# Kainmueller-Lab/PatchPerPix

Measured on AMD Instinct MI355X. Metric: Mvoxels/sec assembled (vote_instances), higher is better.
Workload: dtype f16 in, f32 accumulate

## Files before the change

### patchperpix_amd/csrc/ppp_consensus_v3.hip

```cpp
#include <algorithm>

#include "ppp_kernels.hpp"

namespace ppp {

typedef float v2f __attribute__((ext_vector_type(2)));
typedef float v4f __attribute__((ext_vector_type(4)));
typedef const volatile __attribute__((address_space(3))) v4f *lds_v4f_cvp;

static constexpr int V3_WAVES = 1;
static constexpr int S1V3_GROUP = 3;
static constexpr bool s1v3_prefetch(int PX) { return PX >= 9; }
static constexpr int s1v3_minwaves(int PX) { return PX <= 7 ? 3 : 2; }

static constexpr bool s1v3_split(int PX) { return PX <= 7; }
static constexpr int S1V3_CGROUP = 3;

template <int PX, bool FLAT>
struct V3 {
    static constexpr int RX = PX / 2;
    static constexpr int NC = 64 + (FLAT ? 2 : 1) * (PX - 1);
    static constexpr int NT = 64 + (FLAT ? 4 : 2) * (PX - 1);
    static constexpr int NACC = 2 * PX - 1;
    static constexpr int NEL = PX * NC;
    static constexpr int NIT = (NEL + 63) / 64;
    static constexpr int NELP = NIT * 64;
    static constexpr int FOLD = 255 / PX;
};

__device__ __forceinline__ v2f pk_mul_clamp(v2f a, v2f b) {
    v2f d;
    asm("v_pk_mul_f32 %0, %1, %2 clamp" : "=v"(d) : "v"(a), "v"(b));
    return d;
}
__device__ __forceinline__ v2f pk_fma_clamp(v2f a, v2f b, v2f c) {
    v2f d;
    asm("v_pk_fma_f32 %0, %1, %2, %3 clamp" : "=v"(d) : "v"(a), "v"(b), "v"(c));
    return d;
}
__device__ __forceinline__ v2f pk_nadd_clamp(v2f a, v2f c) {
    v2f d;
    asm("v_pk_add_f32 %0, %1, %2 neg_lo:[1,0] neg_hi:[1,0] clamp" : "=v"(d) : "v"(a), "v"(c));
    return d;
}
__device__ __forceinline__ v2f pk_fma(v2f a, v2f b, v2f c) { return __builtin_elementwise_fma(a, b, c); }
__device__ __forceinline__ uint32_t pk_mad_u16(uint32_t a, uint32_t b, uint32_t c) {
    uint32_t d;
    asm("v_pk_mad_u16 %0, %1, %2, %3" : "=v"(d) : "v"(a), "v"(b), "v"(c));
    return d;
}
__device__ __forceinline__ v2f splat(float x) { return (v2f){x, x}; }
__device__ __forceinline__ uint32_t pack_codes(v2f pos, v2f neg) {
    const v2f c = pk_fma(neg, splat(256.0f), pos);
    return (uint32_t)c.x | ((uint32_t)c.y << 16);
}

template <int PX, int NC, bool ROW0, bool EXACT>
__device__ __forceinline__ void tile_votes3(const v2f *at, const v2f *cfp, lds_v4f_cvp bt, const v2f *bt2, const uint32_t *ct,
                                            const double th2, const double den,
                                            v2f (&acc)[2 * PX - 1], uint32_t (&tc)[2 * PX - 1]) {
    const v2f kq = splat(-0.25f), c43 = splat(0x1.555556p+0f), c43lo = splat(-0x1.555556p-25f);
    constexpr int GS = S1V3_GROUP;
    constexpr int NJG = (PX + GS - 1) / GS;
    constexpr int NG = PX * NJG;
    v4f bcur[GS], bnxt[GS];
    v2f ta, ta_nxt, fa, fa_nxt, ga, na;
    uint32_t ca = 0u;
    lds_v4f_cvp btg[GS];
#pragma unroll
    for (int g = 0; g < GS; ++g) btg[g] = bt;
    auto used = [](int kx, int j) { return j < PX && !(ROW0 && j <= kx); };
    auto load_group = [&](int n, v4f (&b)[GS], v2f &t, v2f &f) {
        const int kx = PX - 1 - n / NJG, jg = (n % NJG) * GS;
        if (jg == 0) { t = at[kx * NC - kx]; f = cfp[-kx]; }
#pragma unroll
        for (int g = 0; g < GS; ++g)
            if (used(kx, jg + g)) {
                if constexpr (s1v3_split(PX)) {
                    const v2f t2 = bt2[(jg + g) * NC - kx];
                    b[g] = (v4f){t2.x, t2.y, __uint_as_float(ct[(jg + g) * NC - kx]), 0.0f};
                } else {
                    b[g] = btg[g][(jg + g) * NC - kx];
                }
            }
    };
    load_group(0, bcur, ta, fa);
#pragma unroll
    for (int n = 0; n < NG; ++n) {
        const int kx = PX - 1 - n / NJG, jg = (n % NJG) * GS;
        if (n + 1 < NG) load_group(n + 1, bnxt, ta_nxt, fa_nxt);
        if (jg == 0) {
            if constexpr (EXACT) ta = (v2f){fa.x != 0.0f ? ta.x : 0.0f, fa.y != 0.0f ? ta.y : 0.0f};
            else ta = ta * fa;
            if constexpr (!EXACT) {
                ga = pk_mul_clamp(ta, splat(4.0f));
                na = pk_mul_clamp(ta, splat(-4.0f));
            } else {
                ga = (v2f){ta.x > 0.0f ? 1.0f : 0.0f, ta.y > 0.0f ? 1.0f : 0.0f};
                na = (v2f){ta.x < 0.0f ? 1.0f : 0.0f, ta.y < 0.0f ? 1.0f : 0.0f};
            }
            ca = pack_codes(ga, na);
        }
        v2f tb[GS], x[GS], y[GS];
        uint32_t cb[GS];
#pragma unroll
        for (int g = 0; g < GS; ++g) {
            if (!used(kx, jg + g)) continue;
            tb[g] = (v2f){bcur[g].x, bcur[g].y};
            cb[g] = __float_as_uint(bcur[g].z);
            x[g] = ta * tb[g];
        }
        if constexpr (!EXACT) {
            v2f dp[GS], dn[GS], d[GS], q0[GS];
#pragma unroll
            for (int g = 0; g < GS; ++g) if (used(kx, jg + g)) dp[g] = pk_fma_clamp(x[g], ga, kq);
#pragma unroll
            for (int g = 0; g < GS; ++g) if (used(kx, jg + g)) dn[g] = pk_nadd_clamp(x[g], kq);
#pragma unroll
            for (int g = 0; g < GS; ++g) if (used(kx, jg + g)) d[g] = dp[g] - dn[g];
#pragma unroll
            for (int g = 0; g < GS; ++g) if (used(kx, jg + g)) q0[g] = d[g] * c43lo;
#pragma unroll
            for (int g = 0; g < GS; ++g) if (used(kx, jg + g)) y[g] = pk_fma(d[g], c43, q0[g]);
        } else {
#pragma unroll
            for (int g = 0; g < GS; ++g) {
                if (!used(kx, jg + g)) continue;
#pragma unroll
                for (int s = 0; s < 2; ++s) {
                    const float a = s ? ta.y : ta.x, b = s ? tb[g].y : tb[g].x, xs = s ? x[g].y : x[g].x;
                    const bool valid = a != 0.0f && b != 0.0f && !(a < 0.0f && b < 0.0f);
                    const double xd = (double)xs;
                    const float ys = (float)((xd - __builtin_copysign(th2, xd)) / den);
                    if (s) y[g].y = valid ? ys : 0.0f; else y[g].x = valid ? ys : 0.0f;
                }
            }
        }
#pragma unroll
        for (int g = 0; g < GS; ++g) {
            if (!used(kx, jg + g)) continue;
            const int i = jg + g - kx + PX - 1;
            acc[i] = acc[i] + y[g];
            tc[i] = pk_mad_u16(ca, cb[g], tc[i]);
        }
        if (n + 1 < NG) {
#pragma unroll
            for (int g = 0; g < GS; ++g) bcur[g] = bnxt[g];
            if ((n + 1) % NJG == 0) { ta = ta_nxt; fa = fa_nxt; }
        }
        __builtin_amdgcn_sched_barrier(0);
    }
}

typedef __amdgpu_buffer_rsrc_t BufRsrc;
__device__ __forceinline__ BufRsrc buf_rsrc(const void *base) {
    return __builtin_amdgcn_make_buffer_rsrc(const_cast<void *>(base), 0, -1, 0x00020000);
}
template <typename T>
__device__ __forceinline__ unsigned buf_ldraw(BufRsrc r, unsigned voff, unsigned soff);
template <>
__device__ __forceinline__ unsigned buf_ldraw<float>(BufRsrc r, unsigned voff, unsigned soff) {
    return __builtin_amdgcn_raw_buffer_load_b32(r, (int)voff, (int)soff, 0);
}
template <>
__device__ __forceinline__ unsigned buf_ldraw<__half>(BufRsrc r, unsigned voff, unsigned soff) {
    return (unsigned)__builtin_amdgcn_raw_buffer_load_b16(r, (int)voff, (int)soff, 0);
}
template <>
__device__ __forceinline__ unsigned buf_ldraw<bf16_t>(BufRsrc r, unsigned voff, unsigned soff) {
    return (unsigned)__builtin_amdgcn_raw_buffer_load_b16(r, (int)voff, (int)soff, 0);
}
template <typename T>
__device__ __forceinline__ unsigned glb_ldraw(const T *base, unsigned voff, unsigned soff);
template <>
__device__ __forceinline__ unsigned glb_ldraw<float>(const float *base, unsigned voff, unsigned soff) {
    asm volatile("" : "+v"(voff));
    return *reinterpret_cast<const unsigned *>(reinterpret_cast<const char *>(base) + soff + voff);
}
template <>
__device__ __forceinline__ unsigned glb_ldraw<__half>(const __half *base, unsigned voff, unsigned soff) {
    asm volatile("" : "+v"(voff));
    return (unsigned)*reinterpret_cast<const unsigned short *>(reinterpret_cast<const char *>(base) + soff + voff);
}
template <>
__device__ __forceinline__ unsigned glb_ldraw<bf16_t>(const bf16_t *base, unsigned voff, unsigned soff) {
    asm volatile("" : "+v"(voff));
    return (unsigned)*reinterpret_cast<const unsigned short *>(reinterpret_cast<const char *>(base) + soff + voff);
}
template <typename T>
__device__ __forceinline__ float widen(unsigned raw);
template <>
__device__ __forceinline__ float widen<float>(unsigned raw) { return __uint_as_float(raw); }
template <>
__device__ __forceinline__ float widen<__half>(unsigned raw) {
    return (float)__builtin_bit_cast(_Float16, (unsigned short)raw);
}
template <>
__device__ __forceinline__ float widen<bf16_t>(unsigned raw) { return __uint_as_float(raw << 16); }

template <typename T>
__device__ __forceinline__ float ldf_at3(const T *base, unsigned byte_off) {
    asm volatile("" : "+v"(byte_off));
    return ldf(reinterpret_cast<const T *>(reinterpret_cast<const char *>(base) + byte_off), 0);
}

enum { V3_DENSE = 0, V3_LIST = 1, V3_ZERO = 2 };

template <typename T, int PX, bool FLAT, bool CLEAN, int MODE = V3_DENSE>
__global__ void __launch_bounds__(64 * V3_WAVES, s1v3_minwaves(PX))
    consensus_v3_kernel(const T *__restrict__ pred, const uint8_t *__restrict__ ov,
                        float *__restrict__ cons, float *__restrict__ cnt_out, const Geo G,
                        const int n_rows, const int runs_per_line, const int bZ2,
                        const long long n_waves, const uint32_t *__restrict__ items) {
    using K = V3<PX, FLAT>;
    constexpr int NIT = K::NIT;
    constexpr bool SPLIT = s1v3_split(PX);
    constexpr bool VOTES = MODE != V3_ZERO;
    __shared__ v4f lds_bt[V3_WAVES][SPLIT || !VOTES ? 1 : K::NELP];
    __shared__ v2f lds_bt2[V3_WAVES][SPLIT && VOTES ? K::NELP : 1];
    __shared__ uint32_t lds_ct[V3_WAVES][SPLIT && VOTES ? K::NELP : 1];
    __shared__ v2f lds_at[V3_WAVES][VOTES ? K::NELP : 1];
    __shared__ v2f lds_cf[V3_WAVES][VOTES ? K::NC : 1];
    __shared__ uint8_t lds_valid[V3_WAVES][2][2][VOTES ? K::NT + 2 : 1];
    const int wave = __builtin_amdgcn_readfirstlane(threadIdx.x >> 6), lane = threadIdx.x & 63;
    long long bid = blockIdx.x;
    {
        const long long nb = gridDim.x, per = nb / 8, main = per * 8;
        if (bid < main) bid = (bid % 8) * per + bid / 8;
    }
    const long long pos = bid * V3_WAVES + wave;
    if (pos >= n_waves) return;
    long long wid_;
    if constexpr (MODE != V3_DENSE) wid_ = (long long)items[pos]; else wid_ = pos;
    const long long wid = wid_;
    const int row = (int)(wid % n_rows);
    long long run = wid / n_rows;
    int dz, dy;
    if (row < G.py) { dz = 0; dy = row; }
    else { const int t = row - G.py; dz = 1 + t / G.wy; dy = t % G.wy - (G.py - 1); }
    const int xr = (int)(run % runs_per_line);
    run /= runs_per_line;
    int uy, uz, ux0, nA;
    if (FLAT) {
        const int flat0 = xr * 64;
        uy = G.cy0 + flat0 / G.cX;
        uz = G.cz0 + 2 * (int)run;
        ux0 = G.cx0 + flat0 % G.cX;
        nA = min(64, G.cX - flat0 % G.cX);
    } else {
        uy = G.cy0 + (int)(run % G.cY);
        uz = G.cz0 + 2 * (int)(run / G.cY);
        ux0 = G.cx0 + xr * 64;
        nA = 64;
    }
    const bool have_s1 = uz + 1 < G.cz0 + G.cZ;
    const bool in_b = FLAT && lane >= nA;
    const bool have_b = FLAT && nA < 64 && uy + 1 < G.cy0 + G.cY;
    const int ux = in_b ? G.cx0 + (lane - nA) : ux0 + lane;
    const int uy_l = in_b ? uy + 1 : uy;
    const bool lane_ok = in_b ? have_b : ux < G.cx0 + G.cX;
    const int pos_l = lane + (PX - 1) + (in_b ? PX - 1 : 0);
    const int wy = uy + dy;
    const bool wy_ok_a = wy >= 0 && wy < G.Y;
    const bool wy_ok_b = have_b && wy + 1 >= 0 && wy + 1 < G.Y;
    const bool wz_ok0 = uz + dz < G.Z, wz_ok1 = have_s1 && uz + 1 + dz < G.Z;
    const bool w_row_ok = (wy_ok_a || wy_ok_b) && (wz_ok0 || wz_ok1);
    const bool row0 = dz == 0 && dy == 0;

    v2f acc[K::NACC];
    uint32_t tc[K::NACC], cnt[K::NACC];
#pragma unroll
    for (int i = 0; i < K::NACC; ++i) { acc[i] = splat(0.0f); tc[i] = 0u; cnt[i] = 0u; }

    const T *mid = pred + (long long)G.mid * G.V;
    const int ntA = nA + 2 * (PX - 1);
    if constexpr (VOTES) {
#pragma unroll
    for (int s = 0; s < 2; ++s) {
        uint8_t *uval = lds_valid[wave][s][0], *wval = lds_valid[wave][s][1];
        const bool s_ok = s == 0 || have_s1;
        const bool wz_ok = s ? wz_ok1 : wz_ok0;
        for (int i = lane; i < K::NT; i += 64) {
            const bool sb = FLAT && i >= ntA;
            const int x = sb ? G.cx0 - (PX - 1) + (i - ntA) : ux0 - (PX - 1) + i;
            const int yy = sb ? uy + 1 : uy, wyy = sb ? wy + 1 : wy;
            bool vu = false, vw = false;
            if (s_ok && x >= 0 && x < G.X && (!sb || have_b)) {
                const long long lu = vox(G, uz + s, yy, x);
                vu = ldf(mid, lu) > G.th_gt && (!G.use_overlap || ov[lu] == 0);
                if (wz_ok && (sb ? wy_ok_b : wy_ok_a)) {
                    const long long lw = vox(G, uz + s + dz, wyy, x);
                    vw = ldf(mid, lw) > G.th_gt && (!G.use_overlap || ov[lw] == 0);
                }
            }
            uval[i] = vu; wval[i] = vw;
        }
    }
    __builtin_amdgcn_fence(__ATOMIC_ACQ_REL, "wavefront");
    __builtin_amdgcn_wave_barrier();
    }

    unsigned el_off[NIT];
    const int ncA = nA + (PX - 1);
    auto centre_x = [&](int i, bool &sb, bool &ok) -> int {
        sb = FLAT && i >= ncA;
        const int iseg = sb ? i - ncA : i;
        const int cx = (sb ? G.cx0 : ux0) - (PX - 1) + K::RX + iseg;
        ok = cx >= K::RX && cx < G.X - K::RX && (!sb || have_b);
        return min(max(cx, 0), G.X - 1) + (sb ? G.X : 0);
    };
#pragma unroll
    for (int it = 0; it < NIT; ++it) {
        const int e = it * 64 + lane;
        const int i = e % K::NC;
        const int j = min(e / K::NC, PX - 1);
        bool sb, ok;
        const int cxc = centre_x(i, sb, ok);
        el_off[it] = (unsigned)(((long long)j * G.V + cxc) * (long long)sizeof(T));
    }
    unsigned cf_off[2];
    unsigned cf_st = 0, cf_sb = 0;
#pragma unroll
    for (int c = 0; c < 2; ++c) {
        const int i = min(lane + 64 * c, K::NC - 1);
        bool sb, ok;
        const int cxc = centre_x(i, sb, ok);
        cf_off[c] = (unsigned)cxc * (unsigned)sizeof(T);
        cf_st |= ((ok && lane + 64 * c < K::NC) ? 1u : 0u) << c;
        cf_sb |= (sb ? 1u : 0u) << c;
    }

    v2f *at = lds_at[wave], *cf = lds_cf[wave];
    v4f *bt = lds_bt[wave];
    v2f *bt2 = lds_bt2[wave];
    uint32_t *ct = lds_ct[wave];

    if (VOTES && w_row_ok) {
        const int kz_hi = min(G.pz - 1, G.pz - 1 - dz), kz_lo = max(0, -dz);
        const int ky_hi = min(G.py - 1, G.py - 1 - dy), ky_lo = max(0, -dy);
        const long long slice = (long long)G.Y * G.X;
        int kz = kz_hi, ky = ky_hi + 1;
        bool row_a_ok = true, row_b_ok = false;
        bool z_ok0 = true, z_ok1 = false;
        auto next_tile = [&](int &z, int &y) -> bool {
            while (true) {
                if (--y < ky_lo) { y = ky_hi; --z; }
                if (z < kz_lo) return false;
                const int cz = uz - z + G.rz, cy = uy - y + G.ry;
                z_ok0 = cz >= G.rz && cz < G.Z - G.rz;
                z_ok1 = have_s1 && cz + 1 >= G.rz && cz + 1 < G.Z - G.rz;
                if (!(z_ok0 || z_ok1)) continue;
                row_a_ok = cy >= G.ry && cy < G.Y - G.ry;
                row_b_ok = have_b && cy + 1 >= G.ry && cy + 1 < G.Y - G.ry;
                if (row_a_ok || row_b_ok) return true;
            }
        };
        unsigned ra[2][NIT], rb[2][NIT], rc[2][2];
        bool lz0 = true, lz1 = false, la = true, lb = false;
        auto load_tile = [&](int z, int y) {
            lz0 = z_ok0; lz1 = z_ok1; la = row_a_ok; lb = row_b_ok;
            const int cz = uz - z + G.rz;
            const long long crow0 = vox(G, z_ok0 ? cz : cz + 1, uy - y + G.ry, 0);
            const unsigned s1 = __builtin_amdgcn_readfirstlane((z_ok1 && z_ok0) ? (unsigned)(slice * (long long)sizeof(T)) : 0u);
            const long long cha = (long long)((z * G.py + y) * PX) * G.V;
            const long long chb = (long long)(((z + dz) * G.py + (y + dy)) * PX) * G.V;
            const BufRsrc qc = buf_rsrc(mid + crow0);
#pragma unroll
            for (int it = 0; it < NIT; ++it) {
                ra[0][it] = glb_ldraw<T>(pred + cha + crow0, el_off[it], 0u);
                ra[1][it] = glb_ldraw<T>(pred + cha + crow0, el_off[it], s1);
                rb[0][it] = glb_ldraw<T>(pred + chb + crow0, el_off[it], 0u);
                rb[1][it] = glb_ldraw<T>(pred + chb + crow0, el_off[it], s1);
            }
#pragma unroll
            for (int c = 0; c < 2; ++c) {
                rc[0][c] = buf_ldraw<T>(qc, cf_off[c], 0u);
                rc[1][c] = buf_ldraw<T>(qc, cf_off[c], s1);
            }
        };
        constexpr bool PREFETCH = s1v3_prefetch(PX);
        const v2f big26 = splat(0x1p26f), nbig26 = splat(-0x1p26f), hb = splat(0x1p25f),
                  nhb = splat(-0x1p25f);
        int n_fold = 0;
        bool have = next_tile(kz, ky);
        if (PREFETCH && have) load_tile(kz, ky);
        while (have) {
            if (!PREFETCH) load_tile(kz, ky);
#pragma unroll
            for (int c = 0; c < 2; ++c) {
                const bool st = (cf_st >> c) & 1u, sb = (cf_sb >> c) & 1u;
                const bool rok = st && (sb ? lb : la);
                v2f f;
                f.x = (rok && lz0 && widen<T>(rc[0][c]) > G.th_gt) ? 1.0f : 0.0f;
                f.y = (rok && lz1 && widen<T>(rc[1][c]) > G.th_gt) ? 1.0f : 0.0f;
                if (lane + 64 * c < K::NC) cf[lane + 64 * c] = f;
            }
            unsigned bigmax = 0u;
            constexpr int CG = S1V3_CGROUP;
#pragma unroll
            for (int it = 0; it < NIT; ++it)
                asm volatile("" : "+v"(ra[0][it]), "+v"(ra[1][it]), "+v"(rb[0][it]), "+v"(rb[1][it]));
            bool any_big = false;
            if constexpr (CLEAN) {
                const v2f c255 = splat(255.0f), one = splat(1.0f);
#pragma unroll
                for (int i0 = 0; i0 < NIT; i0 += CG) {
                    v2f va[CG], vb[CG], ha[CG], hbb[CG], ta[CG], tb[CG], cc[CG];
#pragma unroll
                    for (int q = 0; q < CG; ++q) if (i0 + q < NIT) {
                        va[q] = (v2f){widen<T>(ra[0][i0 + q]), widen<T>(ra[1][i0 + q])};
                        vb[q] = (v2f){widen<T>(rb[0][i0 + q]), widen<T>(rb[1][i0 + q])};
                    }
#pragma unroll
                    for (int q = 0; q < CG; ++q) if (i0 + q < NIT) ha[q] = pk_fma_clamp(va[q], nbig26, hb);
#pragma unroll
                    for (int q = 0; q < CG; ++q) if (i0 + q < NIT) hbb[q] = pk_fma_clamp(vb[q], nbig26, hb);
#pragma unroll
                    for (int q = 0; q < CG; ++q) if (i0 + q < NIT) ta[q] = va[q] - ha[q];
#pragma unroll
                    for (int q = 0; q < CG; ++q) if (i0 + q < NIT) tb[q] = vb[q] - hbb[q];
#pragma unroll
                    for (int q = 0; q < CG; ++q) if (i0 + q < NIT) cc[q] = pk_fma(hbb[q], c255, one);
#pragma unroll
                    for (int q = 0; q < CG; ++q) if (i0 + q < NIT) {
                        const int e = (i0 + q) * 64 + lane;
                        const uint32_t code = (uint32_t)cc[q].x | ((uint32_t)cc[q].y << 16);
                        at[e] = ta[q];
                        if constexpr (SPLIT) { bt2[e] = tb[q]; ct[e] = code; }
                        else bt[e] = (v4f){tb[q].x, tb[q].y, __uint_as_float(code), 0.0f};
                    }
                }
            } else {
#pragma unroll
            for (int i0 = 0; i0 < NIT; i0 += CG) {
                v2f va[CG], vb[CG], ga[CG], ha[CG], gb[CG], hbb[CG], sa[CG], sbb[CG], ta[CG], tb[CG], cc[CG];
#pragma unroll
                for (int q = 0; q < CG; ++q) if (i0 + q < NIT) {
                    va[q] = (v2f){widen<T>(ra[0][i0 + q]), widen<T>(ra[1][i0 + q])};
                    vb[q] = (v2f){widen<T>(rb[0][i0 + q]), widen<T>(rb[1][i0 + q])};
                }
#pragma unroll
                for (int q = 0; q < CG; ++q) if (i0 + q < NIT) ga[q] = pk_fma_clamp(va[q], big26, nhb);
#pragma unroll
                for (int q = 0; q < CG; ++q) if (i0 + q < NIT) ha[q] = pk_fma_clamp(va[q], nbig26, hb);
#pragma unroll
                for (int q = 0; q < CG; ++q) if (i0 + q < NIT) gb[q] = pk_fma_clamp(vb[q], big26, nhb);
#pragma unroll
                for (int q = 0; q < CG; ++q) if (i0 + q < NIT) hbb[q] = pk_fma_clamp(vb[q], nbig26, hb);
#pragma unroll
                for (int q = 0; q < CG; ++q) if (i0 + q < NIT) sa[q] = ga[q] + ha[q];
#pragma unroll
                for (int q = 0; q < CG; ++q) if (i0 + q < NIT) sbb[q] = gb[q] + hbb[q];
#pragma unroll
                for (int q = 0; q < CG; ++q) if (i0 + q < NIT) cc[q] = pk_fma(hbb[q], splat(256.0f), gb[q]);
#pragma unroll
                for (int q = 0; q < CG; ++q) if (i0 + q < NIT) ta[q] = pk_fma(va[q], sa[q], -ha[q]);
#pragma unroll
                for (int q = 0; q < CG; ++q) if (i0 + q < NIT) tb[q] = pk_fma(vb[q], sbb[q], -hbb[q]);
#pragma unroll
                for (int q = 0; q < CG; ++q) if (i0 + q < NIT) {
                    const int e = (i0 + q) * 64 + lane;
                    bigmax = max(bigmax, max(max(__float_as_uint(va[q].x), __float_as_uint(va[q].y)),
                                             max(__float_as_uint(vb[q].x), __float_as_uint(vb[q].y))));
                    const uint32_t code = (uint32_t)cc[q].x | ((uint32_t)cc[q].y << 16);
                    at[e] = ta[q];
                    if constexpr (SPLIT) { bt2[e] = tb[q]; ct[e] = code; }
                    else bt[e] = (v4f){tb[q].x, tb[q].y, __uint_as_float(code), 0.0f};
                }
            }
            any_big = __ballot(bigmax > 0x3F800000u) != 0ull;
            if (any_big) {
#pragma unroll
                for (int it = 0; it < NIT; ++it) {
                    const int e = it * 64 + lane;
                    v2f ta, tb;
                    unsigned code = 0u;
#pragma unroll
                    for (int s = 0; s < 2; ++s) {
                        const float va = widen<T>(ra[s][it]), vb = widen<T>(rb[s][it]);
                        const float xa = va > G.th_gt ? va : (va < G.bg_lt ? va - 1.0f : 0.0f);
                        const float xb = vb > G.th_gt ? vb : (vb < G.bg_lt ? vb - 1.0f : 0.0f);
                        if (s) { ta.y = xa; tb.y = xb; } else { ta.x = xa; tb.x = xb; }
                        code |= (xb > 0.0f ? 1u : (xb < 0.0f ? 256u : 0u)) << (16 * s);
                    }
                    at[e] = ta;
                    if constexpr (SPLIT) { bt2[e] = tb; ct[e] = code; }
                    else bt[e] = (v4f){tb.x, tb.y, __uint_as_float(code), 0.0f};
                }
            }
            }
            __builtin_amdgcn_fence(__ATOMIC_ACQ_REL, "wavefront");
            __builtin_amdgcn_wave_barrier();
            have = next_tile(kz, ky);
            if (PREFETCH && have) load_tile(kz, ky);
            const v2f *ia = at + pos_l;
            lds_v4f_cvp ib = (lds_v4f_cvp)(bt + (SPLIT ? 0 : pos_l));
            const v2f *ib2 = bt2 + (SPLIT ? pos_l : 0);
            const uint32_t *ic = ct + (SPLIT ? pos_l : 0);
            const v2f *icf = cf + pos_l;
            if (CLEAN || !any_big) {
                if (row0) tile_votes3<PX, K::NC, true, false>(ia, icf, ib, ib2, ic, G.th2, G.den, acc, tc);
                else tile_votes3<PX, K::NC, false, false>(ia, icf, ib, ib2, ic, G.th2, G.den, acc, tc);
            } else if constexpr (!CLEAN) {
                if (row0) tile_votes3<PX, K::NC, true, true>(ia, icf, ib, ib2, ic, G.th2, G.den, acc, tc);
                else tile_votes3<PX, K::NC, false, true>(ia, icf, ib, ib2, ic, G.th2, G.den, acc, tc);
            }
            if (++n_fold == K::FOLD) {
                n_fold = 0;
#pragma unroll
                for (int i = 0; i < K::NACC; ++i) {
                    cnt[i] += (tc[i] & 0x00FF00FFu) + ((tc[i] >> 8) & 0x00FF00FFu);
                    tc[i] = 0u;
                }
            }
            __builtin_amdgcn_fence(__ATOMIC_ACQ_REL, "wavefront");
            __builtin_amdgcn_wave_barrier();
        }
    }
    if (!lane_ok) return;
    __builtin_amdgcn_fence(__ATOMIC_ACQ_REL, "wavefront");
    __builtin_amdgcn_wave_barrier();
    const int ti_u = (in_b ? ntA + (lane - nA) : lane) + PX - 1;
#pragma unroll
    for (int s = 0; s < 2; ++s) {
        if (s == 1 && !have_s1) break;
        const uint8_t *uval = lds_valid[wave][s][0], *wval = lds_valid[wave][s][1];
        const bool u_ok = VOTES && uval[ti_u] != 0;
        float val[K::NACC];
#pragma unroll
        for (int i = 0; i < K::NACC; ++i) {
            const int dx = i - (PX - 1);
            val[i] = 0.0f;
            if (dz == 0 && dy == 0 && dx <= 0) continue;
            const unsigned total = cnt[i] + (tc[i] & 0x00FF00FFu) + ((tc[i] >> 8) & 0x00FF00FFu);
            const bool ok = VOTES && u_ok && wval[ti_u + dx] != 0;
            const unsigned n = ok ? ((s ? total >> 16 : total) & 0xFFFFu) : 0u;
            const float a = ok ? (s ? acc[i].y : acc[i].x) : 0.0f;
            const float c = (float)n;
            val[i] = (G.normalise && n != 0u) ? a / c : a;
            if (G.layout != PPP_CONS_VOXEL_MAJOR) {
                const long long o = cons_at(G, dz, dy, dx, uz + s, uy_l, ux);
                if (cons) cons[o] = val[i];
                if (cnt_out) cnt_out[o] = c;
            }
        }
        if (G.layout == PPP_CONS_VOXEL_MAJOR) {
            const int W = (2 * G.pz - 1) * G.wy * G.wx, Lc = (W - 1) / 2;
            const int L0 = (dz * G.wy + dy) * G.wx;
            const long long vu = ((long long)row_slice(G, uz + s) * G.bY + (uy_l - G.by0)) * G.bX + (ux - G.bx0);
            float *pos = cons + vu * W + Lc + L0 - (PX - 1);
            if (row0) {
                pos[PX - 1] = 0.0f;
#pragma unroll
                for (int i = PX; i < K::NACC; ++i) pos[i] = val[i];
            } else {
                typedef float f4u __attribute__((ext_vector_type(4), aligned(4)));
#pragma unroll
                for (int i = 0; i + 4 <= K::NACC; i += 4)
                    *reinterpret_cast<f4u *>(pos + i) = (f4u){val[i], val[i + 1], val[i + 2], val[i + 3]};
#pragma unroll
                for (int i = K::NACC / 4 * 4; i < K::NACC; ++i) pos[i] = val[i];
            }
            const int wz = uz + s + dz, wy2 = uy_l + dy;
            if (wz < G.bz0 + G.bZ && wy2 >= G.by0 && wy2 < G.by0 + G.bY) {
                const long long vw0 = ((long long)row_slice(G, wz) * G.bY + (wy2 - G.by0)) * G.bX + (ux - G.bx0);
#pragma unroll
                for (int i = 0; i < K::NACC; ++i) {
                    const int dx = i - (PX - 1);
                    if (row0 && dx <= 0) continue;
                    const int wx2 = ux + dx;
                    if (wx2 >= G.bx0 && wx2 < G.bx0 + G.bX) cons[(vw0 + dx) * W + Lc - L0 - dx] = val[i];
                }
            }
        }
    }
}

struct VmFaces { long long start[6]; int lo[5][3], ext[5][3]; };
__global__ void __launch_bounds__(256)
    vm_zero_kernel(float *__restrict__ S, const Geo G, const int n_rows, const VmFaces F) {
    const long long t = (long long)blockIdx.x * blockDim.x + threadIdx.x;
    if (t >= F.start[5] * n_rows) return;
    const int row = (int)(t % n_rows);
    const long long fv = t / n_rows;
    int f = 0;
#pragma unroll
    for (int k = 1; k < 5; ++k) f += fv >= F.start[k] ? 1 : 0;
    const long long r = fv - F.start[f];
    const int ex = F.ext[f][2], ey = F.ext[f][1];
    const int bx = F.lo[f][2] + (int)(r % ex), by = F.lo[f][1] + (int)((r / ex) % ey),
              bz = F.lo[f][0] + (int)(r / ((long long)ex * ey));
    int dz, dy;
    if (row < G.py) { dz = 0; dy = row; }
    else { const int q = row - G.py; dz = 1 + q / G.wy; dy = q % G.wy - (G.py - 1); }
    const int W = (2 * G.pz - 1) * G.wy * G.wx, Lc = (W - 1) / 2;
    float *Sv = S + (((long long)bz * G.bY + by) * G.bX + bx) * W;
    const bool line_out = bz - dz < 0 || by - dy < 0 || by - dy >= G.bY;
    const int L0 = (dz * G.wy + dy) * G.wx;
    for (int dx = -(G.px - 1); dx <= G.px - 1; ++dx) {
        if (row == 0 && dx <= 0) continue;
        const int sx = bx - dx;
        if (line_out || sx < 0 || sx >= G.bX) Sv[Lc - L0 - dx] = 0.0f;
    }
}

static hipError_t launch_vm_zero(float *S, const Geo &G, int n_rows, hipStream_t s) {
    VmFaces F{};
    const int gz = std::min(G.pz - 1, G.bZ), gy = std::min(G.py - 1, G.bY), gx = std::min(G.px - 1, G.bX);
    const int lo[5][3] = {{0, 0, 0}, {0, 0, 0}, {0, G.bY - gy, 0}, {0, 0, 0}, {0, 0, G.bX - gx}};
    const int ext[5][3] = {{gz, G.bY, G.bX}, {G.bZ, gy, G.bX}, {G.bZ, gy, G.bX}, {G.bZ, G.bY, gx}, {G.bZ, G.bY, gx}};
    long long acc = 0;
    for (int f = 0; f < 5; ++f) {
        F.start[f] = acc;
        for (int a = 0; a < 3; ++a) { F.lo[f][a] = lo[f][a]; F.ext[f][a] = std::max(ext[f][a], 1); }
        acc += (long long)ext[f][0] * ext[f][1] * ext[f][2];
    }
    F.start[5] = acc;
    const long long nt = acc * n_rows;
    if (nt == 0) return hipSuccess;
    PPP_GRID_CHECK((nt + 255) / 256, 256);
    vm_zero_kernel<<<dim3((unsigned)((nt + 255) / 256)), dim3(256), 0, s>>>(S, G, n_rows, F);
    return hipGetLastError();
}

template <typename T, int PX, bool FLAT, bool CLEAN>
static hipError_t launch_v3f(const T *pred, const uint8_t *ov, float *cons, float *cnt,
                             const Geo &G, hipStream_t s) {
    const int n_rows = (G.pz - 1) * G.wy + G.py;
    const int runs_per_line = FLAT ? (int)(((long long)G.cX * G.cY + 63) / 64) : (G.cX + 63) / 64;
    const int bZ2 = (G.cZ + 1) / 2;
    const long long n_waves = (long long)runs_per_line * (FLAT ? 1 : G.cY) * bZ2 * n_rows;
    const long long n_blocks = (n_waves + V3_WAVES - 1) / V3_WAVES;
    if (n_blocks >= (1ll << 31)) return hipErrorInvalidValue;
    PPP_GRID_CHECK(n_blocks, 64 * V3_WAVES);
    if (((long long)(PX - 1) * G.V + 2ll * G.X) * (long long)sizeof(T) >= (1ll << 32)) return hipErrorNotSupported;
    if (G.layout == PPP_CONS_VOXEL_MAJOR && !G.vm_open) {
        const hipError_t ez = launch_vm_zero(cons, G, n_rows, s);
        if (ez != hipSuccess) return ez;
    }
    consensus_v3_kernel<T, PX, FLAT, CLEAN><<<dim3((unsigned)n_blocks), dim3(64 * V3_WAVES), 0, s>>>(
        pred, ov, cons, cnt, G, n_rows, runs_per_line, bZ2, n_waves, nullptr);
    return hipGetLastError();
}

template <typename T, int PX, bool FLAT, bool CLEAN>
static hipError_t launch_v3f_lists(const T *pred, const uint8_t *ov, float *cons, float *cnt, const Geo &G,
                                   const uint32_t *active, long long n_active, const uint32_t *inactive,
                                   long long n_inactive, hipStream_t s) {
    const int n_rows = (G.pz - 1) * G.wy + G.py;
    const int runs_per_line = FLAT ? (int)(((long long)G.cX * G.cY + 63) / 64) : (G.cX + 63) / 64;
    const int bZ2 = (G.cZ + 1) / 2;
    const long long n_waves = (long long)runs_per_line * (FLAT ? 1 : G.cY) * bZ2 * n_rows;
    if (n_active + n_inactive != n_waves || n_waves >= (1ll << 32)) return hipErrorInvalidValue;
    if (((long long)(PX - 1) * G.V + 2ll * G.X) * (long long)sizeof(T) >= (1ll << 32)) return hipErrorNotSupported;
    if (G.layout == PPP_CONS_VOXEL_MAJOR && !G.vm_open) {
        const hipError_t ez = launch_vm_zero(cons, G, n_rows, s);
        if (ez != hipSuccess) return ez;
    }
    if (n_active > 0) {
        const long long nb = (n_active + V3_WAVES - 1) / V3_WAVES;
        PPP_GRID_CHECK(nb, 64 * V3_WAVES);
        consensus_v3_kernel<T, PX, FLAT, CLEAN, V3_LIST><<<dim3((unsigned)nb), dim3(64 * V3_WAVES), 0, s>>>(
            pred, ov, cons, cnt, G, n_rows, runs_per_line, bZ2, n_active, active);
        const hipError_t e = hipGetLastError();
        if (e != hipSuccess) return e;
    }
    if (n_inactive > 0) {
        const long long nb = (n_inactive + V3_WAVES - 1) / V3_WAVES;
        PPP_GRID_CHECK(nb, 64 * V3_WAVES);
        consensus_v3_kernel<float, PX, FLAT, true, V3_ZERO><<<dim3((unsigned)nb), dim3(64 * V3_WAVES), 0, s>>>(
            nullptr, nullptr, cons, cnt, G, n_rows, runs_per_line, bZ2, n_inactive, inactive);
    }
    return hipGetLastError();
}

static bool v3_flat(const Geo &G) {
    static EnvSwitch sw("PPP_S1_FLAT");
    const char *e = sw.get();
    bool flat = G.cX >= 64 && G.cX % 64 != 0 && G.py >= 3 && G.cY > 1;
    if (e && e[0] == '0') flat = false;
    if (e && e[0] == '1' && G.cX >= 64 && G.py >= 3) flat = true;
    return flat;
}
static bool v3_clean(const Geo &G) {
    static EnvSwitch swc("PPP_S1_CLEAN");
    const char *ec = swc.get();
    return G.pred_clean == 1 && !(ec && ec[0] == '0');
}

V3Items consensus_v3_items(const Geo &G) {
    V3Items I;
    I.flat = v3_flat(G) ? 1 : 0;
    I.n_rows = (G.pz - 1) * G.wy + G.py;
    I.runs_per_line = I.flat ? (int)(((long long)G.cX * G.cY + 63) / 64) : (G.cX + 63) / 64;
    I.bZ2 = (G.cZ + 1) / 2;
    I.n_runs = (long long)I.runs_per_line * (I.flat ? 1 : G.cY) * I.bZ2;
    I.n_items = I.n_runs * I.n_rows;
    return I;
}

template <typename T, int PX>
static hipError_t launch_v3_lists(const T *pred, const uint8_t *ov, float *cons, float *cnt, const Geo &G,
                                  const uint32_t *act, long long na, const uint32_t *ina, long long ni,
                                  hipStream_t s) {
    const bool flat = v3_flat(G);
    const bool clean = v3_clean(G);
    note_consensus_short_form(clean && na > 0 ? 1 : 0);
    if (clean)
        return flat ? launch_v3f_lists<T, PX, true, true>(pred, ov, cons, cnt, G, act, na, ina, ni, s)
                    : launch_v3f_lists<T, PX, false, true>(pred, ov, cons, cnt, G, act, na, ina, ni, s);
    return flat ? launch_v3f_lists<T, PX, true, false>(pred, ov, cons, cnt, G, act, na, ina, ni, s)
                : launch_v3f_lists<T, PX, false, false>(pred, ov, cons, cnt, G, act, na, ina, ni, s);
}

template <typename T, int PX>
static hipError_t launch_v3(const T *pred, const uint8_t *ov, float *cons, float *cnt,
                            const Geo &G, hipStream_t s) {
    const bool flat = v3_flat(G);
    const bool clean = v3_clean(G);
    note_consensus_short_form(clean ? 1 : 0);
    if (clean)
        return flat ? launch_v3f<T, PX, true, true>(pred, ov, cons, cnt, G, s)
                    : launch_v3f<T, PX, false, true>(pred, ov, cons, cnt, G, s);
    return flat ? launch_v3f<T, PX, true, false>(pred, ov, cons, cnt, G, s)
                : launch_v3f<T, PX, false, false>(pred, ov, cons, cnt, G, s);
}

bool consensus_v3_supported(const Geo &G) {
    static EnvSwitch sw("PPP_S1_V3");
    const char *e = sw.get();
    if (e && e[0] == '0') return false;
    return G.value_rule == PPP_VAL_NORM_PROB_PRODUCT && G.th2 == 0.25 && G.den == 0.75 &&
           G.th_gt == 0.5f && G.bg_lt == 0.5f && (G.px == 3 || G.px == 5 || G.px == 7 || G.px == 9);
}

hipError_t launch_consensus_v3(const void *pred, int dtype, const uint8_t *ov, float *cons,
                               float *cnt, const Geo &G, hipStream_t s) {
    if (!consensus_v3_supported(G)) return hipErrorNotSupported;
    if (G.layout == PPP_CONS_VOXEL_MAJOR && (cnt || !cons)) return hipErrorInvalidValue;
#define PPP_V3_CASE(P)                                                                          \
    case P:                                                                                     \
        return with_pred_type(dtype, [&](auto tag) {                                            \
            using T = PPP_PRED_T(tag);                                                          \
            return launch_v3<T, P>((const T *)pred, ov, cons, cnt, G, s);                       \
        });
    switch (G.px) {
        PPP_V3_CASE(3)
        PPP_V3_CASE(5)
        PPP_V3_CASE(7)
        PPP_V3_CASE(9)
    default:
        return hipErrorNotSupported;
    }
#undef PPP_V3_CASE
}

hipError_t launch_consensus_v3_lists(const void *pred, int dtype, const uint8_t *ov, float *cons, float *cnt,
                                     const Geo &G, const uint32_t *active, long long n_active,
                                     const uint32_t *inactive, long long n_inactive, hipStream_t s) {
    if (!consensus_v3_supported(G)) return hipErrorNotSupported;
    if (G.layout == PPP_CONS_VOXEL_MAJOR && (cnt || !cons)) return hipErrorInvalidValue;
#define PPP_V3_CASE(P)                                                                                       \
    case P:                                                                                                  \
        return with_pred_type(dtype, [&](auto tag) {                                                         \
            using T = PPP_PRED_T(tag);                                                                       \
            return launch_v3_lists<T, P>((const T *)pred, ov, cons, cnt, G, active, n_active, inactive,      \
                                         n_inactive, s);                                                     \
        });
    switch (G.px) {
        PPP_V3_CASE(3)
        PPP_V3_CASE(5)
        PPP_V3_CASE(7)
        PPP_V3_CASE(9)
    default:
        return hipErrorNotSupported;
    }
#undef PPP_V3_CASE
}

}
```

Before: 16.28.

## Stage voxel-major consensus results through LDS for coalesced writes; group dense wave order

For larger patch sizes with voxel-major output, each wave writes its per-lane results into LDS. It then cooperatively stores contiguous vector chunks for both the direct and the mirrored (symmetric) offsets instead of doing per-lane strided stores. It also remaps dense wave indices so that groups of runs sharing a row are scheduled together, which should improve cache locality. The change adds LDS traffic and wave barriers, and the rewritten mirror-write logic carries correctness risk.

```diff
diff --git a/patchperpix_amd/csrc/ppp_consensus_v3.hip b/patchperpix_amd/csrc/ppp_consensus_v3.hip
--- a/patchperpix_amd/csrc/ppp_consensus_v3.hip
+++ b/patchperpix_amd/csrc/ppp_consensus_v3.hip
@@ -14,6 +14,8 @@
 static constexpr int s1v3_minwaves(int PX) { return PX <= 7 ? 3 : 2; }
 
 static constexpr bool s1v3_split(int PX) { return PX <= 7; }
+static constexpr bool s1v3_lds_write(int PX) { return PX >= 7; }
+static constexpr int s1v3_group(int PX) { return PX >= 9 ? 32 : PX >= 7 ? 16 : 0; }
 static constexpr int S1V3_CGROUP = 3;
 
 template <int PX, bool FLAT>
@@ -232,6 +234,13 @@
     if (pos >= n_waves) return;
     long long wid_;
     if constexpr (MODE != V3_DENSE) wid_ = (long long)items[pos]; else wid_ = pos;
+    if constexpr (MODE == V3_DENSE && s1v3_group(PX) > 0) {
+        constexpr int GR = s1v3_group(PX);
+        const long long n_runs = n_waves / n_rows, per = (long long)GR * n_rows;
+        const long long grp = pos / per, rem = pos % per;
+        const int in_grp = (int)min((long long)GR, n_runs - grp * GR);
+        wid_ = (grp * GR + rem % in_grp) * n_rows + rem / in_grp;
+    }
     const long long wid = wid_;
     const int row = (int)(wid % n_rows);
     long long run = wid / n_rows;
@@ -517,7 +526,10 @@
             __builtin_amdgcn_wave_barrier();
         }
     }
-    if (!lane_ok) return;
+    constexpr bool LDSW = VOTES && s1v3_lds_write(PX);
+    static_assert(!LDSW || 64 * K::NACC * sizeof(float) <= sizeof(lds_at[0]), "one slice of results fits the image");
+    const bool vm_lds = LDSW && G.layout == PPP_CONS_VOXEL_MAJOR;
+    if (!lane_ok && !vm_lds) return;
     __builtin_amdgcn_fence(__ATOMIC_ACQ_REL, "wavefront");
     __builtin_amdgcn_wave_barrier();
     const int ti_u = (in_b ? ntA + (lane - nA) : lane) + PX - 1;
@@ -525,7 +537,7 @@
     for (int s = 0; s < 2; ++s) {
         if (s == 1 && !have_s1) break;
         const uint8_t *uval = lds_valid[wave][s][0], *wval = lds_valid[wave][s][1];
-        const bool u_ok = VOTES && uval[ti_u] != 0;
+        const bool u_ok = VOTES && lane_ok && uval[ti_u] != 0;
         float val[K::NACC];
 #pragma unroll
         for (int i = 0; i < K::NACC; ++i) {
@@ -543,6 +555,69 @@
                 if (cons) cons[o] = val[i];
                 if (cnt_out) cnt_out[o] = c;
             }
+        }
+        if constexpr (LDSW) if (vm_lds) {
+            typedef float f4u __attribute__((ext_vector_type(4), aligned(4)));
+            constexpr int NACC = K::NACC, NCH = (NACC + 3) / 4;
+            float *stage = reinterpret_cast<float *>(at);
+            if (s == 1) {
+                __builtin_amdgcn_fence(__ATOMIC_ACQ_REL, "wavefront");
+                __builtin_amdgcn_wave_barrier();
+            }
+            if (lane_ok) {
+#pragma unroll
+                for (int i = 0; i < NACC; ++i) stage[lane * NACC + i] = val[i];
+            }
+            __builtin_amdgcn_fence(__ATOMIC_ACQ_REL, "wavefront");
+            __builtin_amdgcn_wave_barrier();
+            const int W = (2 * G.pz - 1) * G.wy * G.wx, Lc = (W - 1) / 2;
+            const int L0 = (dz * G.wy + dy) * G.wx;
+            const int n_a = FLAT ? nA : min(64, G.cx0 + G.cX - ux0);
+            const int n_b = have_b ? 64 - nA : 0;
+            const int i_lo = row0 ? PX - 1 : 0;
+            const int j_hi = row0 ? PX - 1 : NACC;
+            const int zu = row_slice(G, uz + s), wz = uz + s + dz;
+            const bool wz_in = wz < G.bz0 + G.bZ;
+            const int zw = wz_in ? row_slice(G, wz) : 0;
+#pragma unroll
+            for (int seg = 0; seg < (FLAT ? 2 : 1); ++seg) {
+                const int l0 = seg ? nA : 0, n = seg ? n_b : n_a, x0 = seg ? G.cx0 : ux0, yl = uy + seg;
+                if (n <= 0) continue;
+                float *prow = cons + (((long long)zu * G.bY + (yl - G.by0)) * G.bX + (x0 - G.bx0)) * W + Lc + L0 - (PX - 1);
+                for (int t = lane; t < n * NCH; t += 64) {
+                    const int v = t / NCH, c4 = (t % NCH) * 4;
+                    const float *src = stage + (l0 + v) * NACC + c4;
+                    float *dst = prow + (unsigned)(v * W + c4);
+                    if (c4 >= i_lo && c4 + 4 <= NACC) {
+                        *reinterpret_cast<f4u *>(dst) = (f4u){src[0], src[1], src[2], src[3]};
+                    } else {
+#pragma unroll
+                        for (int e = 0; e < 4; ++e)
+                            if (c4 + e >= i_lo && c4 + e < NACC) dst[e] = src[e];
+                    }
+                }
+                const int wy2 = yl + dy;
+                if (!(wz_in && wy2 >= G.by0 && wy2 < G.by0 + G.bY)) continue;
+                const int nt = n + 2 * (PX - 1), wx0 = x0 - (PX - 1);
+                float *mrow = cons + ((long long)zw * G.bY + (wy2 - G.by0)) * G.bX * W + Lc - L0 - (PX - 1);
+                for (int t = lane; t < nt * NCH; t += 64) {
+                    const int v = t / NCH, c4 = (t % NCH) * 4;
+                    const int wx = wx0 + v;
+                    if (wx < G.bx0 || wx >= G.bx0 + G.bX) continue;
+                    const int q0 = v - 2 * (PX - 1) + c4;
+                    const float *src = stage + (l0 + q0) * NACC + (NACC - 1 - c4);
+                    float *dst = mrow + (unsigned)((wx - G.bx0) * W + c4);
+                    if (q0 >= 0 && q0 + 3 < n && c4 + 4 <= j_hi) {
+                        *reinterpret_cast<f4u *>(dst) =
+                            (f4u){src[0], src[NACC - 1], src[2 * (NACC - 1)], src[3 * (NACC - 1)]};
+                    } else {
+#pragma unroll
+                        for (int e = 0; e < 4; ++e)
+                            if (q0 + e >= 0 && q0 + e < n && c4 + e < j_hi) dst[e] = src[e * (NACC - 1)];
+                    }
+                }
+            }
+            continue;
         }
         if (G.layout == PPP_CONS_VOXEL_MAJOR) {
             const int W = (2 * G.pz - 1) * G.wy * G.wx, Lc = (W - 1) / 2;
```

Result: no change. 16.50, median of 4 (+1.4%).
